# kylittle/Crucible

Hardware: AMD Instinct MI355X
Metric: Msamples/sec (whole node) + achieved HBM GB/s, book1 1920×1080 @ 1/2/4/8 GPU (higher is better)
Workload: dtype f64

## Files before the change

### crucible_amd/csrc/pathtrace.hpp

```cpp
#pragma once
#include <hip/hip_runtime.h>
#include <stddef.h>
#include <stdint.h>
#include <type_traits>

#define CR_HD __host__ __device__ __forceinline__
#define CR_D __device__ __forceinline__
#include "fastdiv.hpp"
#include "residency.hpp"

namespace cr {

template <typename real> struct RealTraits;
template <> struct RealTraits<float> {
    static constexpr float eps = 1.1920928955078125e-07f;
    static constexpr float tiny = 0.0f;
    static constexpr float pi = 3.14159265358979323846f;
};
template <> struct RealTraits<double> {
    static constexpr double eps = 2.220446049250313e-16;
    static constexpr double tiny = 1e-160;
    static constexpr double pi = 3.14159265358979323846;
};

// ... 599 lines not shown
    }
}
template <typename real> CR_D void random_in_unit_disk_dev(uint64_t& s, real& px, real& py) {
    if constexpr (!std::is_same<real, double>::value) {
        for (;;) {
            px = rng_range<real>(s, real(-1), real(1));
            py = rng_range<real>(s, real(-1), real(1));
            if (px * px + py * py + real(0) * real(0) < real(1)) break;
        }
    } else {
        uint64_t ux, uy;
        for (;;) {
            ux = rng_next(s); uy = rng_next(s);
            const float fx = screen_coord(ux), fy = screen_coord(uy);
            const float lf = __builtin_fmaf(fy, fy, fx * fx);
            if (lf > 1.0f + 1e-5f) continue;
            if (lf < 1.0f - 1e-5f) break;
            const double x = -1.0 + 2.0 * u01(ux, 0.0), y = -1.0 + 2.0 * u01(uy, 0.0);
            if (x * x + y * y + 0.0 * 0.0 < 1.0) break;
        }
        px = -1.0 + 2.0 * u01(ux, 0.0); py = -1.0 + 2.0 * u01(uy, 0.0);
    }
}

template <typename real, bool ANIM, bool CAMK = false>
CR_D void camera_ray(const KernelArgs<real>& A, uint32_t pix_i, uint32_t pix_j, int32_t sample, uint64_t& rng, V3<real>& ro, V3<real>& rd,
                     real& rtime, real current_time) {
    const CamConst<real>& cam = A.cam;
    uint32_t pixel = pix_j * (uint32_t)cam.W + pix_i;
    rng = rng_key(A.seed_mixed, pixel, (uint32_t)sample);
    real ts = current_time + rng_range<real>(rng, real(0), A.shutter_length);
    real ox = rng_uniform<real>(rng) - real(0.5);
    real oy = rng_uniform<real>(rng) - real(0.5);
    CamFrame<real> f;
    if ((ANIM || CAMK) && cam.animated) {
        real fx = cam.from.x, fy = cam.from.y, fz = cam.from.z, fw = real(1);
        real ax = cam.at.x, ay = cam.at.y, az = cam.at.z, aw = real(1);
        timeline_eval(A.cam_keys + cam.from_key_first, cam.from_key_count, ts, fx, fy, fz, fw);
        timeline_eval(A.cam_keys + cam.at_key_first, cam.at_key_count, ts, ax, ay, az, aw);
        f = camera_frame(cam, mk<real>(fw * fx, fw * fy, fw * fz), mk<real>(aw * ax, aw * ay, aw * az));
    } else {
        f.from = cam.from; f.p00 = cam.p00; f.pdu = cam.pdu; f.pdv = cam.pdv; f.ddu = cam.ddu; f.ddv = cam.ddv;
    }
    V3<real> ps = add(add(f.p00, scale((real)pix_i + ox, f.pdu)), scale((real)pix_j + oy, f.pdv));
    V3<real> orig = f.from;
    if (cam.defocus_on) {
        real px, py;
        random_in_unit_disk_dev<real>(rng, px, py);
        orig = add(add(f.from, scale(px, f.ddu)), scale(py, f.ddv));
    }
    ro = orig; rd = sub(ps, orig); rtime = ts;
}
template <typename real, bool ANIM, bool CAMK = false>
CR_D void camera_ray(const KernelArgs<real>& A, uint32_t pix_i, uint32_t pix_j, int32_t sample, uint64_t& rng, V3<real>& ro, V3<real>& rd,
                     real& rtime) {
    camera_ray<real, ANIM, CAMK>(A, pix_i, pix_j, sample, rng, ro, rd, rtime, A.current_time);
}

template <typename T> CR_D T load_rec(const T* p, bool in_lds) {
    static_assert(sizeof(T) % 4 == 0, "records are whole words");
    T out;
    uint32_t* o = reinterpret_cast<uint32_t*>(&out);
    if (in_lds) {
        const __attribute__((address_space(3))) uint32_t* s = (const __attribute__((address_space(3))) uint32_t*)(const void*)p;
        for (size_t k = 0; k < sizeof(T) / 4; k++) o[k] = s[k];
    } else {
        const __attribute__((address_space(1))) uint32_t* s = (const __attribute__((address_space(1))) uint32_t*)(const void*)p;
        for (size_t k = 0; k < sizeof(T) / 4; k++) o[k] = s[k];
    }
    return out;
}

#define CR_CHECKER_LEAF(tex_at, ti, tx, p)                                                                                          \
    for (int guard = 0; guard < 32 && tx.kind == 1; guard++) {                                                                   \
        int32_t s = (int32_t)((uint32_t)as_i32(r_floor(tx.inv_scale * p.x)) + (uint32_t)as_i32(r_floor(tx.inv_scale * p.y)) +   \
                              (uint32_t)as_i32(r_floor(tx.inv_scale * p.z)));                                                      \
        ti = (s % 2 == 0) ? tx.even : tx.odd;                                                                                    \
        tx = tex_at(ti);                                                                                                         \
    }

template <typename real, bool ANIM, bool SIDE_SPLIT = false, bool RELAX = false>
CR_D bool shade(const KernelArgs<real>& A, const Prim<real>* prims, const Mat<real>* mats, const Tex<real>* texs, V3<real>& ro, V3<real>& rd,
                real rtime, uint64_t& rng, int32_t& depth_left, int32_t& stack_n, real best_t, int32_t best, uint32_t stack_stride,
                uint32_t stack_slot, uint32_t& c_tex, V3<real>& col, Diag* dg = nullptr, V3<real>* thr = nullptr) {
    CR_DIAG_HIT(dg, DG_SHADE_WAVE, DG_SHADE_LANE);
    if (best >= 0) {
        CR_DIAG_HIT(dg, DG_HITSH_WAVE, DG_HITSH_LANE);
        const Prim<real>& p = prims[best];
        V3<real> loc = add(ro, scale(best_t, rd));
        V3<real> n;
        real tu = 0, tv = 0;
        auto mat_at = [&](int32_t i) { return SIDE_SPLIT ? load_rec(mats + i, A.lds_side != 0) : mats[i]; };
        auto tex_at = [&](int32_t i) { return SIDE_SPLIT ? load_rec(texs + i, A.lds_side != 0) : texs[i]; };
        const Mat<real> m = mat_at(p.mat());
        bool need_uv = false;
        int32_t leaf_tex = -1;
        if (m.kind == 0 && m.tex >= 0) {
            int ti = m.tex;
            Tex<real> tx = tex_at(ti);
            CR_CHECKER_LEAF(tex_at, ti, tx, loc)
            need_uv = tx.kind == 2;
            leaf_tex = ti;
        }
        if (p.kind() == 0) {
            real g0 = p.g[0], g1 = p.g[1], g2 = p.g[2], g3 = p.g[3];
            if (ANIM && p.key_count) {
                timeline_eval(A.keys + p.key_first, p.key_count, rtime, g0, g1, g2, g3);
                n = divs(sub(loc, mk<real>(g0, g1, g2)), g3);
            } else n = scale(p.g[4], sub(loc, mk<real>(g0, g1, g2)));
            if (need_uv) {
                real theta = r_acos(-n.y);
                real phi = r_atan2(-n.z, n.x) + RealTraits<real>::pi;
                tu = phi / (real(2) * RealTraits<real>::pi);
                tv = theta / RealTraits<real>::pi;
            }
        } else {
            V3<real> a = mk<real>(p.g[0], p.g[1], p.g[2]), b = mk<real>(p.g[3], p.g[4], p.g[5]), c = mk<real>(p.g[6], p.g[7], p.g[8]);
            if (ANIM && p.key_count) {
                a = timeline_vertex(A.keys + p.key_first, p.key_count, rtime, a);
                b = timeline_vertex(A.keys + p.key_first, p.key_count, rtime, b);
                c = timeline_vertex(A.keys + p.key_first, p.key_count, rtime, c);
            }
            n = unit(cross(sub(b, a), sub(c, a)));
            tu = 0; tv = 0;
        }
        bool front = dot(rd, n) < real(0);
        if (!front) n = neg(n);

        V3<real> att = mk<real>(0, 0, 0), ndir = rd;
        bool some;
        V3<real> ruv = mk<real>(0, 0, 0);
#ifdef CR_DIAG
        if (m.kind != 2) {
            for (;;) {
                CR_DIAG_HIT(dg, DG_RUV_WAVE, DG_RUV_LANE);
                real x = rng_range<real>(rng, real(-1), real(1)), y = rng_range<real>(rng, real(-1), real(1)), z = rng_range<real>(rng, real(-1), real(1));
                V3<real> pp = mk<real>(x, y, z);
                real lensq = len2(pp);
                if (RealTraits<real>::tiny < lensq && lensq <= real(1)) { ruv = divs(pp, r_sqrt(lensq)); break; }
            }
        }
        CR_DIAG_LANE(dg, m.kind == 0 ? DG_LAMB_LANE : (m.kind == 1 ? DG_METAL_LANE : DG_DIEL_LANE));
#else
        if (m.kind != 2) ruv = random_unit_vector_dev<real>(rng);
#endif
        if (m.kind == 0) {
            V3<real> dir = add(n, ruv);
            real tol = real(1e-8);
            if (r_abs(dir.x) < tol && r_abs(dir.y) < tol && r_abs(dir.z) < tol) dir = n;
            V3<real> tc;
            if (m.tex < 0) tc = mk<real>(m.albedo[0], m.albedo[1], m.albedo[2]);
            else {
                const Tex<real> lt = tex_at(leaf_tex);
                if (need_uv) tc = image_lookup(A.images, A.texels, lt.image, tu, tv, c_tex);
                else tc = mk<real>(lt.color[0], lt.color[1], lt.color[2]);
            }
            att = c_scale(m.aux, (m.param < real(0)) ? c_neg(tc) : tc);
            ndir = dir;
            if (__ballot(!(m.param >= real(1))) == 0ull) { rng_step(rng); some = true; }
            else some = rng_uniform<real>(rng) <= m.param;
        } else if (m.kind == 1) {
            V3<real> refl = reflect(rd, n);
            refl = add(unit(refl), scale(m.param, ruv));
            att = mk<real>(m.albedo[0], m.albedo[1], m.albedo[2]);
            ndir = refl;
            some = dot(refl, n) > real(0);
        } else {
            att = mk<real>(1, 1, 1);
            real ri = front ? m.albedo[0] : m.param;
            V3<real> ud = unit(rd);
            real cos_theta = -(r_fmin(dot(ud, n), real(1)));
            real sin_theta = r_sqrt(real(1) - cos_theta * cos_theta);
            bool refl = ri * sin_theta > real(1);
            if (!refl) {
                real r0 = front ? m.albedo[1] : m.albedo[2];
                real x = real(1) - cos_theta;
                real x2 = x * x;
                real x5 = x * (x2 * x2);
                refl = (r0 + (real(1) - r0) * x5) > rng_uniform<real>(rng);
            }
            ndir = refl ? reflect(ud, n) : refract(ud, n, ri);
            some = true;
        }
        if (!some) { col = mk<real>(0, 0, 0); return true; }
        if (m.kind != 2) {
            if constexpr (RELAX) { thr->x = thr->x * att.x; thr->y = thr->y * att.y; thr->z = thr->z * att.z; }
            else {
                real* rec = A.att_stack + ((size_t)stack_n * stack_stride + stack_slot) * 3;
                rec[0] = att.x; rec[1] = att.y; rec[2] = att.z;
                stack_n++;
            }
        }
        ro = loc; rd = ndir; depth_left--;
        return false;
    }
    CR_DIAG_LANE(dg, DG_SKY_LANE);
    V3<real> ud = unit(rd);
    if (A.sky_kind == 1) {
        real theta = r_atan2(ud.x, ud.z);
        real phi = r_asin(ud.y);
        real u = (theta / (real(2) * RealTraits<real>::pi)) + real(0.5);
        real v = (phi / RealTraits<real>::pi) + real(0.5);
        col = image_lookup(A.images, A.texels, A.sky_image, u, v, c_tex);
    } else {
        real a = real(0.5) * (ud.y + real(1));
        col = c_add(c_scale(real(1) - a, mk<real>(1, 1, 1)), c_scale(a, mk<real>(real(0.5), real(0.7), real(1))));
    }
    if constexpr (RELAX) { col = mk<real>(thr->x * col.x, thr->y * col.y, thr->z * col.z); return true; }
    int32_t k = stack_n - 1;
    for (; k >= 3; k -= 4) {
        CR_DIAG_HIT(dg, DG_UNWIND_WAVE, DG_UNWIND_LANE);
        V3<real> a[4];
#pragma unroll
        for (int j = 0; j < 4; j++) {
            const real* rec = A.att_stack + ((size_t)(k - j) * stack_stride + stack_slot) * 3;
            a[j] = mk<real>(rec[0], rec[1], rec[2]);
        }
#pragma unroll
        for (int j = 0; j < 4; j++) col = c_mul(a[j], col);
    }
    for (; k >= 0; k--) {
        CR_DIAG_HIT(dg, DG_UNWIND_WAVE, DG_UNWIND_LANE);
        const real* rec = A.att_stack + ((size_t)k * stack_stride + stack_slot) * 3;
        V3<real> a_k = mk<real>(rec[0], rec[1], rec[2]);
        col = c_mul(a_k, col);
    }
    return true;
}

template <typename T> using LdsPtr = const __attribute__((address_space(3))) T*;
template <typename T> using GlobPtr = const __attribute__((address_space(1))) T*;
template <typename real, int RES>
CR_D Entry<real> fetch_entry(const Entry<real>* lds, const Entry<real>* glob, int32_t lds_entries, int32_t idx) {
    if (RES == RES_LDS) return lds[idx];
    if (RES == RES_TOP) {
        Entry<real> e;
        if (idx < lds_entries) {
            const Entry<real>* s = lds + idx;
            LdsPtr<real> b = (LdsPtr<real>)s->b;
            for (int k = 0; k < 6; k++) e.b[k] = b[k];
            e.skip = *(LdsPtr<int32_t>)&s->skip; e.leaf = *(LdsPtr<int32_t>)&s->leaf;
        } else {
            const Entry<real>* s = glob + idx;
            GlobPtr<real> b = (GlobPtr<real>)s->b;
            for (int k = 0; k < 6; k++) e.b[k] = b[k];
            e.skip = *(GlobPtr<int32_t>)&s->skip; e.leaf = *(GlobPtr<int32_t>)&s->leaf;
        }
        return e;
    }
    return glob[idx];
}
template <typename real, int RES>
CR_D Entry<real> fetch_entry_ordered(const Entry<real>* lds, const Entry<real>* glob, int32_t lds_entries, int32_t idx, int32_t oct) {
    auto rd = [&](const EntryO<real>* p) {
        const EntryO<real>& s = p[idx];
        Entry<real> e;
        for (int k = 0; k < 6; k++) e.b[k] = s.b[k];
        e.leaf = s.leaf;
        e.skip = s.skip[oct];
        return e;
    };
    if (RES == RES_LDS) return rd((const EntryO<real>*)lds);
    if (RES == RES_TOP) {
        Entry<real> e;
        if (idx < lds_entries) {
            const EntryO<real>* s = (const EntryO<real>*)lds + idx;
            LdsPtr<real> b = (LdsPtr<real>)s->b;
            for (int k = 0; k < 6; k++) e.b[k] = b[k];
            e.leaf = *(LdsPtr<int32_t>)&s->leaf; e.skip = ((LdsPtr<int32_t>)s->skip)[oct];
        } else {
            const EntryO<real>* s = (const EntryO<real>*)glob + idx;
            GlobPtr<real> b = (GlobPtr<real>)s->b;
            for (int k = 0; k < 6; k++) e.b[k] = b[k];
            e.leaf = *(GlobPtr<int32_t>)&s->leaf; e.skip = ((GlobPtr<int32_t>)s->skip)[oct];
        }
        return e;
    }
    return rd((const EntryO<real>*)glob);
}

template <int RES> CR_D uint32_t screen_lds_base(const void* lds) { return RES == RES_LDS ? (uint32_t)(uintptr_t)(LdsPtr<char>)lds : 0u; }
template <int RES>
CR_D ScreenEntry fetch_screen(const ScreenEntry* lds, const ScreenEntry* glob, uint32_t lds_bytes, uint32_t off) {
    static_assert(sizeof(ScreenEntry) == 32, "offsets are index << 5");
    typedef uint32_t Quad __attribute__((ext_vector_type(4)));
    if (RES == RES_LDS) {
        ScreenEntry e;
        Quad* o = reinterpret_cast<Quad*>(&e);
        LdsPtr<Quad> s = (LdsPtr<Quad>)(uintptr_t)off;
        o[0] = s[0]; o[1] = s[1];
        return e;
    }
    if (RES == RES_TOP) {
        ScreenEntry e;
        Quad* o = reinterpret_cast<Quad*>(&e);
        if (off < lds_bytes) {
            LdsPtr<Quad> s = (LdsPtr<Quad>)(const void*)((const char*)lds + off);
            o[0] = s[0]; o[1] = s[1];
        } else {
            GlobPtr<Quad> s = (GlobPtr<Quad>)(const void*)((const char*)glob + off);
            o[0] = s[0]; o[1] = s[1];
        }
        return e;
    }
    return *(const ScreenEntry*)((const char*)glob + off);
}

struct ScreenStepO { float b[6]; uint32_t axis, hit, skip; };
template <int RES>
CR_D ScreenStepO fetch_screen_ordered(const ScreenEntryO* lds, const ScreenEntryO* glob, uint32_t lds_bytes, uint32_t off, uint32_t octoff) {
    static_assert(sizeof(ScreenEntryO) == 64, "offsets are index << 6");
    typedef uint32_t Quad __attribute__((ext_vector_type(4)));
    ScreenStepO e;
    Quad q0, q1;
    if (RES == RES_LDS) {
        LdsPtr<Quad> s = (LdsPtr<Quad>)(uintptr_t)off;
        q0 = s[0]; q1 = s[1];
        e.skip = *(LdsPtr<uint32_t>)(uintptr_t)(off + octoff);
    } else if (RES == RES_TOP && off < lds_bytes) {
        LdsPtr<Quad> s = (LdsPtr<Quad>)(const void*)((const char*)lds + off);
        q0 = s[0]; q1 = s[1];
        e.skip = *(LdsPtr<uint32_t>)(const void*)((const char*)lds + off + octoff);
    } else {
        GlobPtr<Quad> s = (GlobPtr<Quad>)(const void*)((const char*)glob + off);
        q0 = s[0]; q1 = s[1];
        e.skip = *(GlobPtr<uint32_t>)(const void*)((const char*)glob + off + octoff);
    }
    uint32_t w[8];
    __builtin_memcpy(w, &q0, 16); __builtin_memcpy(w + 4, &q1, 16);
    for (int k = 0; k < 6; k++) e.b[k] = __builtin_bit_cast(float, w[k]);
    e.axis = w[6]; e.hit = w[7];
    return e;
}

template <typename real> struct WalkState {
    V3<real> inv;
    real dd;
    real rda;
    real best_t;
    int32_t best;
    int32_t idx;
    bool exact_box;
    int32_t oct;
    int32_t pending;
};

CR_D bool tree_walks_exact(const KernelArgs<float>& A) { return A.exact_boxes != 0; }
CR_D constexpr bool tree_walks_exact(const KernelArgs<double>&) { return false; }

template <bool SHARED = false, typename real> CR_D void walk_begin(WalkState<real>& w, V3<real> rd, bool exact_tree = false) {
    w.inv = mk<real>(real(1) / rd.x, real(1) / rd.y, real(1) / rd.z);
    w.exact_box = exact_tree || (r_abs(w.inv.x) == r_inf(real(0))) || (r_abs(w.inv.y) == r_inf(real(0))) || (r_abs(w.inv.z) == r_inf(real(0)));
    w.dd = len2(rd);
    w.rda = SHARED ? shared_rcp(w.dd) : quot_divide<real>();
    w.idx = 0; w.best_t = r_inf(real(0)); w.best = -1; w.pending = -1;
    w.oct = (rd.x < real(0) ? 1 : 0) | (rd.y < real(0) ? 2 : 0) | (rd.z < real(0) ? 4 : 0);
}

CR_D void screen_extents(float ofx, float ofy, float ofz, float ifx, float ify, float ifz, float& mo, float& pmax, float& pmin) {
    mo = r_max(r_max(__builtin_fabsf(ofx), __builtin_fabsf(ofy)), __builtin_fabsf(ofz));
    pmax = r_max(r_max(__builtin_fabsf(ifx), __builtin_fabsf(ify)), __builtin_fabsf(ifz));
    pmin = r_min(r_min(__builtin_fabsf(ifx), __builtin_fabsf(ify)), __builtin_fabsf(ifz));
}
CR_D bool screen_in_range(bool exact_box, float mo, float pmax, float pmin) {
    return !exact_box && pmin >= 0x1.0p-100f && pmax <= 0x1.0p100f && mo <= 0x1.0p100f;
}
CR_D float screen_q(float of, float inv_f) { return __builtin_fabsf(of * inv_f); }
CR_D float screen_th0(float qx, float qy, float qz, float pmax) {
    return __builtin_fmaf(0x1.0p-20f, r_max(r_max(qx, qy), qz), __builtin_fmaf(pmax * 0x1.0p-100f, 0x1.0p-47f, 1e-35f));
}
CR_D float screen_box_d(const float* b, Pair<float> fox, Pair<float> foy, Pair<float> foz, Pair<float> fix, Pair<float> fiy, Pair<float> fiz,
                        float tminf, float tmaxf, float th0, float& th) {
    const Pair<float> tx = __builtin_elementwise_fma(Pair<float>{b[0], b[1]}, fix, -(fox * fix));
    const Pair<float> ty = __builtin_elementwise_fma(Pair<float>{b[2], b[3]}, fiy, -(foy * fiy));
    const Pair<float> tz = __builtin_elementwise_fma(Pair<float>{b[4], b[5]}, fiz, -(foz * fiz));
    const float nx = r_min(tx.x, tx.y), ny = r_min(ty.x, ty.y), nz = r_min(tz.x, tz.y);
    const float fx = r_max(tx.x, tx.y), fy = r_max(ty.x, ty.y), fz = r_max(tz.x, tz.y);
    const float lo = r_max(r_max(nx, ny), r_max(nz, tminf));
    float hi, m;
    asm("v_min_f32_e32 %0, %2, %3\n\tv_min3_f32 %0, %4, %5, %0\n\tv_max_f32_e64 %1, |%6|, |%0|"
        : "=&v"(hi), "=v"(m) : "v"(fz), "v"(tmaxf), "v"(fx), "v"(fy), "v"(lo));
    th = __builtin_fmaf(0x1.0p-20f, m, th0);
    return hi - lo;
}
CR_D bool screen_box_miss_exact(const float* b, Pair<float> fox, Pair<float> foy, Pair<float> foz, Pair<float> fix, Pair<float> fiy,
                                Pair<float> fiz, float tminf, float tmaxf) {
    const Pair<float> tx = (Pair<float>{b[0], b[1]} - fox) * fix;
    const Pair<float> ty = (Pair<float>{b[2], b[3]} - foy) * fiy;
    const Pair<float> tz = (Pair<float>{b[4], b[5]} - foz) * fiz;
    const float nx = r_min(tx.x, tx.y), ny = r_min(ty.x, ty.y), nz = r_min(tz.x, tz.y);
    const float fx = r_max(tx.x, tx.y), fy = r_max(ty.x, ty.y), fz = r_max(tz.x, tz.y);
    const float lo = r_max(r_max(nx, ny), r_max(nz, tminf));
    float hi;
    asm("v_min_f32_e32 %0, %1, %2\n\tv_min3_f32 %0, %3, %4, %0" : "=&v"(hi) : "v"(fz), "v"(tmaxf), "v"(fx), "v"(fy));
    return hi <= lo;
}

template <typename real, int RES, bool ANIM, bool SCREEN> constexpr int quot_form() {
    constexpr bool fits = std::is_same<real, double>::value && !ANIM && SCREEN && RES != RES_GLOBAL;
#ifdef CR_QUOT_FORM
    return fits ? CR_QUOT_FORM : 0;
#else
    return fits ? 1 : 0;
#endif
}

template <typename real, int RES, bool ANIM, bool ORD = false, bool SCREEN = false, bool SHARE = false>
CR_D void walk_round(const KernelArgs<real>& A, const Entry<real>* lds_entries, const Prim<real>* prims, V3<real> ro, V3<real> rd, real rtime,
                     WalkState<real>& w, bool walking, uint32_t budget, unsigned long long& c_node, uint32_t& c_prim, Diag* dg = nullptr,
                     const void* lds_screen = nullptr) {
    constexpr bool EXACT = std::is_same<real, float>::value;
    static_assert(!(SCREEN && EXACT && ORD), "the f32 kernels use ScreenEntry records for unordered trees only");
    const real tmin = real(0.001);
    const int32_t n_entries = A.n_entries;
    constexpr int RES64 = SCREEN ? RES_GLOBAL : RES;
    const int32_t lds_n64 = SCREEN ? 0 : A.lds_entries;
    int32_t leaf = w.pending;
    if (walking && leaf < 0) {
        CR_DIAG_HIT(dg, DG_ROUND_WAVE, DG_ROUND_LANE);
        uint32_t exact_steps = w.exact_box ? 0xffffffffu : 0u;
        if constexpr (SCREEN) {
            const float ofx = (float)ro.x, ofy = (float)ro.y, ofz = (float)ro.z;
            const float ifx = (float)w.inv.x, ify = (float)w.inv.y, ifz = (float)w.inv.z;
            float mo, pmax, pmin;
            screen_extents(ofx, ofy, ofz, ifx, ify, ifz, mo, pmax, pmin);
            bool screened;
            if constexpr (EXACT) screened = !w.exact_box;
            else screened = screen_in_range(w.exact_box, mo, pmax, pmin);
            if (!screened) exact_steps = 0xffffffffu;
            else {
                const float qx = screen_q(ofx, ifx), qy = screen_q(ofy, ify), qz = screen_q(ofz, ifz);
                const Pair<float> fox = {ofx, ofx}, foy = {ofy, ofy}, foz = {ofz, ofz};
                const Pair<float> fix = {ifx, ifx}, fiy = {ify, ify}, fiz = {ifz, ifz};
                const float tminf = 0.001f;
                float tmaxf = (float)w.best_t;
                const float th0 = screen_th0(qx, qy, qz, pmax);
                asm volatile("" : "+v"(tmaxf));
                uint32_t nodes = 0;
                auto box_miss = [&](const float* b, int32_t idx) -> bool {
                    if constexpr (EXACT) {
                        const bool miss = screen_box_miss_exact(b, fox, foy, foz, fix, fiy, fiz, tminf, tmaxf);
                        nodes++;
                        CR_DIAG_HIT(dg, DG_BOX_WAVE, DG_BOX_LANE);
                        return miss;
                    }
                    float th;
                    float d = screen_box_d(b, fox, foy, foz, fix, fiy, fiz, tminf, tmaxf, th0, th);
                    nodes++;
                    CR_DIAG_HIT(dg, DG_BOX_WAVE, DG_BOX_LANE);
                    const bool band = !(__builtin_fabsf(d) > th);
                    if (__builtin_expect(__ballot(band) != 0ull, 0)) {
                        if (band) {
                            CR_DIAG_HIT(dg, DG_BAND_WAVE, DG_BAND_LANE);
                            const Entry<real> e = ORD ? fetch_entry_ordered<real, RES64>(lds_entries, A.entries, lds_n64, idx, w.oct)
                                                      : fetch_entry<real, RES64>(lds_entries, A.entries, lds_n64, idx);
                            d = box_hit(e.b, ro, w.inv, tmin, w.best_t) ? 1.0f : -1.0f;
                        }
                    }
                    return d < 0.0f;
                };
                if constexpr (ORD) {
                    const uint32_t base = screen_lds_base<RES>(lds_screen);
                    const uint32_t end = base + ((uint32_t)n_entries << 6);
                    const uint32_t oct = (uint32_t)w.oct, octoff = 32u + (oct << 2);
                    uint32_t off = base + ((uint32_t)w.idx << 6), after_leaf = 0;
                    if (off < end) {
                        for (uint32_t it = 0;; it++) {
                            const ScreenStepO se = fetch_screen_ordered<RES>((const ScreenEntryO*)lds_screen, (const ScreenEntryO*)A.screen, (uint32_t)A.lds_entries << 6, off, octoff);
                            const bool miss = box_miss(se.b, (int32_t)((off - base) >> 6));
                            after_leaf = se.skip;
                            off = miss ? se.skip : se.hit + (__builtin_amdgcn_ubfe(oct, se.axis, 1u) << 6);
                            uint32_t limit = (it + 1 == budget) ? 0u : end;
                            asm("" : "+s"(limit));
                            if (off >= limit) break;
                        }
                        if (off & kScreenLeaf) { leaf = (int32_t)(off & ~kScreenLeaf); off = after_leaf; }
                        w.idx = (int32_t)((off - base) >> 6);
                    }
                } else {
                    const uint32_t base = screen_lds_base<RES>(lds_screen);
                    const uint32_t end = base + ((uint32_t)n_entries << 5);
                    uint32_t off = base + ((uint32_t)w.idx << 5), after_leaf = 0;
                    if (off < end) {
                        for (uint32_t it = 0;; it++) {
                            const ScreenEntry se = fetch_screen<RES>((const ScreenEntry*)lds_screen, (const ScreenEntry*)A.screen, (uint32_t)A.lds_entries << 5, off);
                            const bool miss = box_miss(se.b, (int32_t)((off - base) >> 5));
                            after_leaf = se.skip;
                            off = miss ? se.skip : se.hit;
                            uint32_t limit = (it + 1 == budget) ? 0u : end;
                            asm("" : "+s"(limit));
                            if (off >= limit) break;
                        }
                        if (off & kScreenLeaf) { leaf = (int32_t)(off & ~kScreenLeaf); off = after_leaf; }
                        w.idx = (int32_t)((off - base) >> 5);
                    }
                }
                c_node += nodes;
            }
        } else if (!w.exact_box) {
            const Pair<real> ox = {ro.x, ro.x}, oy = {ro.y, ro.y}, oz = {ro.z, ro.z};
            const Pair<real> ix = {w.inv.x, w.inv.x}, iy = {w.inv.y, w.inv.y}, iz = {w.inv.z, w.inv.z};
            const real tmax = w.best_t;
            uint32_t nodes = 0;
            for (uint32_t it = 0; w.idx < n_entries; it++) {
                const Entry<real> e = ORD ? fetch_entry_ordered<real, RES64>(lds_entries, A.entries, lds_n64, w.idx, w.oct)
                                          : fetch_entry<real, RES64>(lds_entries, A.entries, lds_n64, w.idx);
                nodes++;
                CR_DIAG_HIT(dg, DG_BOX_WAVE, DG_BOX_LANE);
                const bool miss = box_miss_fast(e.b, ox, oy, oz, ix, iy, iz, tmin, tmax);
                const bool inner = e.leaf < 0;
                w.idx = (inner && !miss) ? (ORD ? ordered_near(e.leaf, w.oct) : -e.leaf) : e.skip;
                if (!(miss || inner)) { leaf = e.leaf; break; }
                if (it + 1 == budget) break;
            }
            c_node += nodes;
        }
        for (; exact_steps != 0u && w.idx < n_entries; exact_steps--) {
            const Entry<real> e = ORD ? fetch_entry_ordered<real, RES64>(lds_entries, A.entries, lds_n64, w.idx, w.oct)
                                      : fetch_entry<real, RES64>(lds_entries, A.entries, lds_n64, w.idx);
            c_node++;
            bool hit = box_hit(e.b, ro, w.inv, tmin, w.best_t);
            w.idx = (hit && e.leaf < 0) ? (ORD ? ordered_near(e.leaf, w.oct) : -e.leaf) : e.skip;
            if (hit && e.leaf >= 0) { leaf = e.leaf; break; }
        }
    }
    w.pending = leaf;
    if (A.walk_leaf_min > 0u) {
        const uint32_t parked = (uint32_t)__popcll(__ballot(leaf >= 0));
        const bool can_step = __ballot(walking && leaf < 0 && w.idx < n_entries) != 0ull;
        if (parked < A.walk_leaf_min && can_step) return;
    }
    w.pending = -1;
    if (leaf >= 0) {
        CR_DIAG_HIT(dg, DG_LEAFPH_WAVE, DG_LEAFPH_LANE);
        constexpr int QF = SHARE ? quot_form<real, RES, ANIM, SCREEN>() : 0;
        const real ra = QF == 1 ? w.rda : (QF == 2 ? shared_rcp(w.dd) : quot_divide<real>());
        auto test = [&](int32_t pi) {
            const Prim<real>& p = prims[pi];
            c_prim++;
            CR_DIAG_HIT(dg, DG_PRIM_WAVE, DG_PRIM_LANE);
            real t;
            bool h;
            real g0 = p.g[0], g1 = p.g[1], g2 = p.g[2], g3 = p.g[3];
            const int32_t kind = A.uniform_kind >= 0 ? A.uniform_kind : p.kind();
            if (kind == 0) {
                if (ANIM && p.key_count) timeline_eval(A.keys + p.key_first, p.key_count, rtime, g0, g1, g2, g3);
                h = sphere_t<RES == RES_LDS || (std::is_same<real, double>::value && !ANIM), QF != 0>(g0, g1, g2, g3, ro, rd, w.dd, tmin, w.best_t, t, dg, ra);
            } else {
                V3<real> a = mk<real>(g0, g1, g2), b = mk<real>(g3, p.g[4], p.g[5]), c = mk<real>(p.g[6], p.g[7], p.g[8]);
                if (ANIM && p.key_count) {
                    a = timeline_vertex(A.keys + p.key_first, p.key_count, rtime, a);
                    b = timeline_vertex(A.keys + p.key_first, p.key_count, rtime, b);
                    c = timeline_vertex(A.keys + p.key_first, p.key_count, rtime, c);
                }
                h = triangle_t(a, b, c, ro, rd, tmin, w.best_t, t);
            }
            if (h) { w.best_t = t; w.best = pi; }
        };
        if (!ANIM || A.leaf_runs == nullptr || !(leaf & kLeafRun)) {
            const int32_t first = leaf >> 1, count = (leaf & 1) + 1;
            if constexpr (RES != RES_LDS && !ANIM) {
                constexpr uint32_t touch = sizeof(Prim<real>) == 96 ? 20u : (uint32_t)(sizeof(Prim<real>) / 4 - 1);
                static_assert((touch + 1) * 4 <= sizeof(Prim<real>), "the touched word must lie inside the record");
                GlobPtr<uint32_t> nx = (GlobPtr<uint32_t>)(const void*)(prims + first + (count - 1));
                const uint32_t t0 = nx[0], t1 = nx[touch];
                test(first);
                asm volatile("" :: "v"(t0), "v"(t1));
                if (count == 2) test(first + 1);
            } else
            for (int32_t k = 0; k < count; k++) test(first + k);
        } else {
            const int32_t first = A.leaf_runs[2 * (leaf & kLeafRunIndex)], count = A.leaf_runs[2 * (leaf & kLeafRunIndex) + 1];
            for (int32_t k = 0; k < count; k++) test(first + k);
        }
    }
}

#ifdef CR_DIAG
#define CR_DIAG_ONLY(...) __VA_ARGS__
#else
#define CR_DIAG_ONLY(...)
#endif

enum : int { ST_NEED_PIXEL = 0, ST_NEED_SAMPLE = 1, ST_TRACE = 2, ST_DONE = 3, ST_WALK = 4, ST_SHADE = 5 };

template <typename real> struct MaxBlock { static constexpr int value = 1024; };

CR_D uint32_t wave_rank(uint64_t ballot) {
    return __builtin_amdgcn_mbcnt_hi((uint32_t)(ballot >> 32), __builtin_amdgcn_mbcnt_lo((uint32_t)ballot, 0u));
}

template <typename real> CR_D const KernelArgs<real>& kernel_args() {
    return *(const KernelArgs<real>*)(const __attribute__((address_space(4))) KernelArgs<real>*)__builtin_amdgcn_kernarg_segment_ptr();
}
template <typename real, int RES, bool ANIM, bool ORD, bool CAMK = false, bool RELAX = false, bool SCREEN = false, bool REG = true, bool LIST = false>
CR_D void pathtrace_body(const KernelArgs<real>& A) {
    using EntryT = typename EntryOf<real, ORD>::type;
    constexpr bool BATCH = RELAX && (ANIM || CAMK);
    constexpr bool REGION = BATCH && REG;
    const KernelArgs<real>& RG = kernel_args<real>();
    extern __shared__ __attribute__((aligned(16))) unsigned char smem[];
#ifdef CR_HOLD_VCC
    unsigned long long vcc_hold;
    asm volatile("s_mov_b64 %0, 0" : "={vcc}"(vcc_hold));
#endif
    const Entry<real>* lds_entries = nullptr;
    const void* lds_screen = nullptr;
    const Prim<real>* prims = A.prims;
    const Mat<real>* mats = A.mats;
    const Tex<real>* texs = A.texs;
    if (RES != RES_GLOBAL) {
        auto copy = [&](const void* src, size_t off, size_t bytes) {
            const uint32_t* s = (const uint32_t*)src;
            uint32_t* d = (uint32_t*)(smem + off);
            for (size_t i = threadIdx.x; i < bytes / 4; i += blockDim.x) d[i] = s[i];
        };
        using ScreenT = typename ScreenOf<ORD>::type;
        constexpr size_t window_rec = SCREEN ? sizeof(ScreenT) : sizeof(EntryT);
        copy(SCREEN ? A.screen : (const void*)A.entries, 0, (size_t)A.lds_entries * window_rec);
        lds_entries = (const Entry<real>*)smem;
        if (SCREEN) lds_screen = (const void*)smem;
        if (RES == RES_LDS) {
            size_t o1 = (((size_t)A.n_entries * window_rec + 15) & ~(size_t)15);
            size_t o2 = o1 + (((size_t)A.n_prims * sizeof(Prim<real>) + 15) & ~(size_t)15);
            size_t o3 = o2 + (((size_t)A.n_mats * sizeof(Mat<real>) + 15) & ~(size_t)15);
            copy(A.prims, o1, (size_t)A.n_prims * sizeof(Prim<real>));
            copy(A.mats, o2, (size_t)A.n_mats * sizeof(Mat<real>));
            copy(A.texs, o3, (size_t)A.n_texs * sizeof(Tex<real>));
            prims = (const Prim<real>*)(smem + o1);
            mats = (const Mat<real>*)(smem + o2);
            texs = (const Tex<real>*)(smem + o3);
            if constexpr (SCREEN) {
                __syncthreads();
                const uint32_t base = screen_lds_base<RES>(smem);
                ScreenT* rec = (ScreenT*)smem;
                for (int32_t i = (int32_t)threadIdx.x; i < A.n_entries; i += (int32_t)blockDim.x) {
                    if constexpr (ORD) { for (int k = 0; k < 8; k++) rec[i].skip[k] += base; }
                    else rec[i].skip += base;
                    if (!(rec[i].hit & kScreenLeaf)) rec[i].hit += base;
                }
            }
        } else if (A.lds_side) {
            size_t o2 = (((size_t)A.lds_entries * window_rec + 15) & ~(size_t)15);
            size_t o3 = o2 + (((size_t)A.n_mats * sizeof(Mat<real>) + 15) & ~(size_t)15);
            copy(A.mats, o2, (size_t)A.n_mats * sizeof(Mat<real>));
            copy(A.texs, o3, (size_t)A.n_texs * sizeof(Tex<real>));
            mats = (const Mat<real>*)(smem + o2);
            texs = (const Tex<real>*)(smem + o3);
        }
        __syncthreads();
    }

    const uint32_t lane = threadIdx.x & 63u;
    const uint32_t gtid = blockIdx.x * blockDim.x + threadIdx.x;
    constexpr uint32_t kFxNoTile = 0xffffffffu;
    unsigned long long* fx_slots = nullptr;
    uint32_t fx_tile0 = kFxNoTile, fx_tile1 = kFxNoTile, fx_mru = 0;
    V3<real> thr = mk<real>(1, 1, 1);
    const uint32_t fx_words = 3u << (A.sg_lw + A.sg_lh);
    if constexpr (RELAX) {
        fx_slots = (unsigned long long*)(smem + A.fx_lds_off) + (size_t)(threadIdx.x >> 6) * 2 * fx_words;
        for (uint32_t k = lane; k < 2 * fx_words; k += 64) fx_slots[k] = 0ull;
        __builtin_amdgcn_fence(__ATOMIC_SEQ_CST, "wavefront");
    }
    auto fx_flush = [&](uint32_t slot, uint32_t tile) {
        if constexpr (RELAX) {
            __builtin_amdgcn_fence(__ATOMIC_SEQ_CST, "wavefront");
            if (tile != kFxNoTile) {
                uint32_t ti, tj;
                tile_xy(A, tile, ti, tj);
                ti <<= A.sg_lw; tj <<= A.sg_lh;
                if constexpr (BATCH) tj -= batch_frame(A, tj) * ((A.tiles_y << A.sg_lh) - (REGION ? RG.reg_h : (uint32_t)A.cam.H));
                for (uint32_t k = lane; k < fx_words; k += 64) {
                    unsigned long long* w = fx_slots + slot * fx_words + k;
                    const unsigned long long v = *w;
                    if (v) {
                        *w = 0ull;
                        const uint32_t px = k / 3u, ch = k - px * 3u;
                        const uint32_t pi = ti + (px & ((1u << A.sg_lw) - 1u)), pj = tj + (px >> A.sg_lw);
                        unsigned long long* g;
                        if constexpr (REGION) g = A.fx_acc + ((size_t)pj * (size_t)RG.reg_w + pi) * 3 + ch;
                        else g = A.fx_acc + ((size_t)pj * (size_t)A.cam.W + pi) * 3 + ch;
                        if (v & ~kFxNaN) atomicAdd(g, v & ~kFxNaN);
                        if (v & kFxNaN) atomicOr(g, kFxNaN);
                    }
                }
            }
            __builtin_amdgcn_fence(__ATOMIC_SEQ_CST, "wavefront");
        }
    };
    const uint32_t total_work = (A.sg_on || RELAX) ? A.sg_total : A.tiles_x * A.tiles_y * 64u;
    const CamConst<real>& cam = A.cam;
    uint32_t wv_next = 0, wv_end = 0;
    const uint32_t SG_CHUNK = A.sg_chunk;

    int state = ST_NEED_PIXEL;
    uint32_t pix_i = 0, pix_j = 0;
    uint32_t item = 0;
    int32_t sample = 0;
    real acc_r = 0, acc_g = 0, acc_b = 0;
    V3<real> ro = mk<real>(0, 0, 0), rd = mk<real>(0, 0, 1);
    real rtime = 0;
    uint64_t rng = 0;
    int32_t depth_left = 0, stack_n = 0;
    uint32_t c_seg = 0, c_prim = 0, c_tex = 0;
    unsigned long long c_node = 0;
    WalkState<real> ws;
    ws.inv = mk<real>(0, 0, 0); ws.dd = 0; ws.rda = quot_divide<real>(); ws.best_t = 0; ws.best = -1; ws.idx = 0; ws.exact_box = false; ws.pending = -1;
    const int32_t n_entries = A.n_entries;
    uint32_t exact_tree = tree_walks_exact(A) ? 1u : 0u;
    if constexpr (std::is_same<real, float>::value) {
        exact_tree = (uint32_t)__builtin_amdgcn_readfirstlane((int)exact_tree);
        asm volatile("" : "+s"(exact_tree));
    }

    Diag* dgp = nullptr;
    CR_DIAG_ONLY(Diag dg_store; for (int i = 0; i < DG_N; i++) dg_store.v[i] = 0; dgp = &dg_store;
                 unsigned long long d_t_regen = 0, d_t_trace = 0, d_t_shade = 0;
                 unsigned long long d_t0 = __builtin_readcyclecounter(); const unsigned long long d_begin = d_t0;)
    for (;;) {
        CR_DIAG_ONLY(if (CR_DIAG_LEADER()) dg_store.v[DG_OUTER_WAVE]++; d_t0 = __builtin_readcyclecounter();)
        uint64_t need = __ballot(state == ST_NEED_PIXEL);
        if (need && (A.sg_on || RELAX)) {
            const uint32_t cnt = (uint32_t)__popcll(need), avail = wv_end - wv_next;
            uint32_t fresh = 0;
            uint32_t my_tile = kFxNoTile;
            if (cnt > avail) {
                const int leader = __ffsll((unsigned long long)need) - 1;
                if ((int)lane == leader) fresh = atomicAdd(A.work_counter, SG_CHUNK);
                fresh = (uint32_t)__builtin_amdgcn_readlane((int)fresh, leader);
            }
            if (state == ST_NEED_PIXEL) {
                const uint32_t rank = wave_rank(need);
                const uint32_t w = rank < avail ? wv_next + rank : fresh + (rank - avail);
                if (w >= total_work) state = ST_DONE;
                else {
                    item = w;
                    const uint32_t group = w >> 6, in = w & 63u;
                    uint32_t tile = fastdiv(group, A.fd_groups);
                    const uint32_t sg = group - tile * A.sg_groups;
                    if constexpr (REGION && LIST) { const int32_t* const listed = RG.tile_list; if (listed) tile = (uint32_t)listed[tile]; }
                    uint32_t tx, ty;
                    tile_xy(A, tile, tx, ty);
                    my_tile = tile;
                    const uint32_t px = in & ((1u << A.sg_lw) - 1u), py = (in >> A.sg_lw) & ((1u << A.sg_lh) - 1u);
                    const uint32_t ds = in >> (A.sg_lw + A.sg_lh);
                    pix_i = (tx << A.sg_lw) + px;
                    pix_j = (ty << A.sg_lh) + py;
                    const uint32_t s_off = sg * (64u >> (A.sg_lw + A.sg_lh)) + ds;
                    sample = (int32_t)((uint32_t)A.sample_begin + s_off);
                    uint32_t row = pix_j;
                    if constexpr (BATCH) row -= batch_frame(A, pix_j) * (A.tiles_y << A.sg_lh);
                    bool inside;
                    if constexpr (REGION) inside = pix_i < RG.reg_w && row < RG.reg_h;
                    else inside = pix_i < (uint32_t)cam.W && row < (uint32_t)cam.H;
                    if (inside && s_off < (uint32_t)(A.sample_end - A.sample_begin)) state = ST_NEED_SAMPLE;
                    if constexpr (REGION) { pix_i += RG.reg_x0; pix_j += RG.reg_y0; }
                }
            }
            if (cnt > avail) { wv_next = fresh + (cnt - avail); wv_end = fresh + SG_CHUNK; }
            else wv_next += cnt;
            if constexpr (RELAX) {
                uint64_t fresh_items = __ballot(state == ST_NEED_SAMPLE) & need;
                while (fresh_items) {
                    const uint32_t t = (uint32_t)__builtin_amdgcn_readlane((int)my_tile, __ffsll((unsigned long long)fresh_items) - 1);
                    fresh_items &= ~__ballot(my_tile == t);
                    if (t == fx_tile0) fx_mru = 0;
                    else if (t == fx_tile1) fx_mru = 1;
                    else if (fx_mru == 0) { fx_flush(1, fx_tile1); fx_tile1 = t; fx_mru = 1; }
                    else { fx_flush(0, fx_tile0); fx_tile0 = t; fx_mru = 0; }                }
            }
        } else if (need) {
            uint32_t cnt = (uint32_t)__popcll(need);
            uint32_t base = 0;
            int leader = __ffsll((unsigned long long)need) - 1;
            if ((int)lane == leader) base = atomicAdd(A.work_counter, cnt);
            base = (uint32_t)__builtin_amdgcn_readlane((int)base, leader);
            if (state == ST_NEED_PIXEL) {
                uint32_t rank = wave_rank(need);
                uint32_t w = base + rank;
                if (w >= total_work) state = ST_DONE;
                else {
                    uint32_t tile = w >> 6, in = w & 63u;
                    uint32_t tx, ty;
                    tile_xy(A, tile, tx, ty);
                    pix_i = tx * 8u + (in & 7u);
                    pix_j = ty * 8u + (in >> 3);
                    if (pix_i < (uint32_t)cam.W && pix_j < (uint32_t)cam.H) {
                        state = ST_NEED_SAMPLE; sample = A.sample_begin; acc_r = acc_g = acc_b = 0;
                    }
                }
            }
        }
        if (__ballot(state != ST_DONE) == 0) break;

        if (state == ST_NEED_SAMPLE) {
            CR_DIAG_HIT(dgp, DG_REGEN_WAVE, DG_REGEN_LANE);
            if constexpr (BATCH) {
                const uint32_t f = batch_frame(A, REGION ? pix_j - RG.reg_y0 : pix_j);
                camera_ray<real, ANIM, CAMK>(A, pix_i, pix_j - f * (A.tiles_y << A.sg_lh), sample, rng, ro, rd, rtime,
                                             A.n_frames > 1u ? A.frame_times[f] : A.current_time);
            } else camera_ray<real, ANIM, CAMK>(A, pix_i, pix_j, sample, rng, ro, rd, rtime);
            depth_left = A.max_depth; stack_n = 0;
            if constexpr (RELAX) thr = mk<real>(1, 1, 1);
            state = ST_TRACE;
        }

        CR_DIAG_ONLY({ unsigned long long t = __builtin_readcyclecounter(); d_t_regen += t - d_t0; d_t0 = t; })
        V3<real> col = mk<real>(0, 0, 0);
        bool finished = false;
        if (state == ST_TRACE) {
            if (depth_left == 0) finished = true;
            else {
                c_seg++;
                walk_begin<quot_form<real, RES, ANIM, SCREEN>() == 1>(ws, rd, exact_tree != 0u);
                state = n_entries > 0 ? ST_WALK : ST_SHADE;
            }
        }
        if (__ballot(state == ST_WALK)) {
            for (;;) {
                walk_round<real, RES, ANIM, ORD, SCREEN, true>(A, lds_entries, prims, ro, rd, rtime, ws, state == ST_WALK, A.walk_round_steps, c_node, c_prim, dgp, lds_screen);
                if (state == ST_WALK && ws.idx >= n_entries && ws.pending < 0) state = ST_SHADE;
                const uint64_t walking = __ballot(state == ST_WALK);
                if (!walking || 64u - (uint32_t)__popcll(walking) >= A.walk_exit_lanes) break;
            }
        }
        const bool tracing = (state == ST_SHADE);

        CR_DIAG_ONLY({ unsigned long long t = __builtin_readcyclecounter(); d_t_trace += t - d_t0; d_t0 = t; })
        if (tracing) {
            finished = shade<real, ANIM, RES == RES_TOP, RELAX>(A, prims, mats, texs, ro, rd, rtime, rng, depth_left, stack_n, ws.best_t, ws.best,
                                         A.n_threads, gtid, c_tex, col, dgp, &thr);
            state = ST_TRACE;
        }

        if (RELAX && finished) {
            if constexpr (RELAX) {
                const bool black = col.x == real(0) && col.y == real(0) && col.z == real(0);
                if (!black) {
                    uint32_t ri = pix_i, rj = pix_j;
                    if constexpr (REGION) { ri -= RG.reg_x0; rj -= RG.reg_y0; }
                    const uint32_t tile = (rj >> A.sg_lh) * A.tiles_x + (ri >> A.sg_lw);
                    const uint32_t px = ((rj & ((1u << A.sg_lh) - 1u)) << A.sg_lw) | (ri & ((1u << A.sg_lw) - 1u));
                    const real cc[3] = {col.x, col.y, col.z};
                    unsigned long long v[3];
#pragma unroll
                    for (int c = 0; c < 3; c++) {
                        const double x = (double)cc[c];
                        v[c] = (x == x) ? (unsigned long long)(__builtin_bit_cast(long long, __builtin_fma(x, A.fx_scale, 0x1.0p52)) - 0x4330000000000000ll) : kFxNaN;
                    }
                    const bool nan = (v[0] | v[1] | v[2]) >> 63;
                    unsigned long long* dst;
                    bool in_lds = true;
                    if (tile == fx_tile0) dst = fx_slots + px * 3u;
                    else if (tile == fx_tile1) dst = fx_slots + fx_words + px * 3u;
                    else {
                        uint32_t row = rj;
                        if constexpr (BATCH) row -= batch_frame(A, rj) * ((A.tiles_y << A.sg_lh) - (REGION ? RG.reg_h : (uint32_t)cam.H));
                        if constexpr (REGION) dst = A.fx_acc + ((size_t)row * (size_t)RG.reg_w + ri) * 3;
                        else dst = A.fx_acc + ((size_t)row * (size_t)cam.W + ri) * 3;
                        in_lds = false;
                    }
                    if (!nan) {
                        if (in_lds) {
                            auto d = (__attribute__((address_space(3))) unsigned long long*)dst;
                            for (int c = 0; c < 3; c++) if (v[c]) (void)__hip_atomic_fetch_add(d + c, v[c], __ATOMIC_RELAXED, __HIP_MEMORY_SCOPE_WORKGROUP);
                        } else {
                            auto d = (__attribute__((address_space(1))) unsigned long long*)dst;
                            for (int c = 0; c < 3; c++) if (v[c]) (void)__hip_atomic_fetch_add(d + c, v[c], __ATOMIC_RELAXED, __HIP_MEMORY_SCOPE_AGENT);
                        }
                    } else {
                        for (int c = 0; c < 3; c++) {
                            if (v[c] >> 63) atomicOr(dst + c, kFxNaN);
                            else if (v[c]) atomicAdd(dst + c, v[c]);
                        }
                    }
                }
            }
            state = ST_NEED_PIXEL;
        } else if (finished && A.sg_on) {
            real* o = A.sample_buf + (size_t)item * 3;
            o[0] = col.x; o[1] = col.y; o[2] = col.z;
            state = ST_NEED_PIXEL;
        } else if (finished) {
            acc_r += col.x; acc_g += col.y; acc_b += col.z;
            sample++;
            if (sample >= A.sample_end) {
                size_t o = ((size_t)pix_j * (size_t)cam.W + pix_i) * 3;
                if (A.output_sum) { A.out[o] = acc_r; A.out[o + 1] = acc_g; A.out[o + 2] = acc_b; }
                else {
                    real cnt = (real)A.samples_total;
                    A.out[o] = acc_r / cnt; A.out[o + 1] = acc_g / cnt; A.out[o + 2] = acc_b / cnt;
                }
                state = ST_NEED_PIXEL;
            } else state = ST_NEED_SAMPLE;
        }
        CR_DIAG_ONLY({ unsigned long long t = __builtin_readcyclecounter(); d_t_shade += t - d_t0; d_t0 = t; })
    }

    if constexpr (RELAX) { fx_flush(0, fx_tile0); fx_flush(1, fx_tile1); }
    auto wave_sum = [&](unsigned long long v) -> unsigned long long {
        unsigned long long s = v;
        for (int off = 32; off > 0; off >>= 1) s += __shfl_down(s, off);
        return s;
    };
    unsigned long long s0 = wave_sum(c_seg), s1 = wave_sum(c_node), s2 = wave_sum(c_prim), s3 = wave_sum(c_tex);
    CR_DIAG_ONLY(
        {
            unsigned long long* c = (unsigned long long*)A.counters;
            for (int i = 0; i < DG_N; i++) { unsigned long long w = wave_sum(dg_store.v[i]); if (lane == 0) atomicAdd(&c[16 + i], w); }
            if (lane == 0) {
                atomicAdd(&c[9], d_t_regen); atomicAdd(&c[10], d_t_trace); atomicAdd(&c[11], d_t_shade);
                atomicAdd(&c[12], __builtin_readcyclecounter() - d_begin);
            }
        })
// ... 85 lines not shown
```

Measured before the change: 4832.

## Compute f64 ray inverse lazily, add sphere leaf loop, reuse squared length in shade

For the f64 screened kernels, the walk now keeps only a float reciprocal of the ray direction, computed with a hardware rcp plus one Newton step. The full double-precision inverse is recomputed on demand, only when exact box tests are needed, instead of being stored in the walk state. It also adds a specialised one-or-two-sphere leaf loop for LDS-resident uniform-sphere scenes. Shade now reuses the squared direction length from the walk state instead of renormalising the ray. The aims are fewer f64 divisions and lower register pressure, at the cost of more template variants and some recomputation on exact fallback paths.

```diff
diff --git a/crucible_amd/csrc/pathtrace.hpp b/crucible_amd/csrc/pathtrace.hpp
--- a/crucible_amd/csrc/pathtrace.hpp
+++ b/crucible_amd/csrc/pathtrace.hpp
@@ -705,8 +705,9 @@
 template <typename real, bool ANIM, bool SIDE_SPLIT = false, bool RELAX = false>
 CR_D bool shade(const KernelArgs<real>& A, const Prim<real>* prims, const Mat<real>* mats, const Tex<real>* texs, V3<real>& ro, V3<real>& rd,
                 real rtime, uint64_t& rng, int32_t& depth_left, int32_t& stack_n, real best_t, int32_t best, uint32_t stack_stride,
-                uint32_t stack_slot, uint32_t& c_tex, V3<real>& col, Diag* dg = nullptr, V3<real>* thr = nullptr) {
+                uint32_t stack_slot, uint32_t& c_tex, V3<real>& col, Diag* dg = nullptr, V3<real>* thr = nullptr, const real* dd = nullptr) {
     CR_DIAG_HIT(dg, DG_SHADE_WAVE, DG_SHADE_LANE);
+    auto unit_rd = [&]() -> V3<real> { return divs(rd, r_sqrt(dd ? *dd : len2(rd))); };
     if (best >= 0) {
         CR_DIAG_HIT(dg, DG_HITSH_WAVE, DG_HITSH_LANE);
         const Prim<real>& p = prims[best];
@@ -791,7 +792,7 @@
         } else {
             att = mk<real>(1, 1, 1);
             real ri = front ? m.albedo[0] : m.param;
-            V3<real> ud = unit(rd);
+            V3<real> ud = unit_rd();
             real cos_theta = -(r_fmin(dot(ud, n), real(1)));
             real sin_theta = r_sqrt(real(1) - cos_theta * cos_theta);
             bool refl = ri * sin_theta > real(1);
@@ -818,7 +819,7 @@
         return false;
     }
     CR_DIAG_LANE(dg, DG_SKY_LANE);
-    V3<real> ud = unit(rd);
+    V3<real> ud = unit_rd();
     if (A.sky_kind == 1) {
         real theta = r_atan2(ud.x, ud.z);
         real phi = r_asin(ud.y);
@@ -956,7 +957,12 @@
     return e;
 }
 
-template <typename real> struct WalkState {
+template <typename real> struct WalkScreened {};
+template <> struct WalkScreened<double> {
+    V3<float> invf;
+    bool unscreened;
+};
+template <typename real> struct WalkState : WalkScreened<real> {
     V3<real> inv;
     real dd;
     real rda;
@@ -979,6 +985,7 @@
     w.idx = 0; w.best_t = r_inf(real(0)); w.best = -1; w.pending = -1;
     w.oct = (rd.x < real(0) ? 1 : 0) | (rd.y < real(0) ? 2 : 0) | (rd.z < real(0) ? 4 : 0);
 }
+template <bool SHARED = false, typename real> CR_D void walk_begin_screened(WalkState<real>& w, V3<real> ro, V3<real> rd);
 
 CR_D void screen_extents(float ofx, float ofy, float ofz, float ifx, float ify, float ifz, float& mo, float& pmax, float& pmin) {
     mo = r_max(r_max(__builtin_fabsf(ofx), __builtin_fabsf(ofy)), __builtin_fabsf(ofz));
@@ -988,9 +995,30 @@
 CR_D bool screen_in_range(bool exact_box, float mo, float pmax, float pmin) {
     return !exact_box && pmin >= 0x1.0p-100f && pmax <= 0x1.0p100f && mo <= 0x1.0p100f;
 }
+CR_D double screen_rcp1(double d) {
+    const double r0 = __builtin_amdgcn_rcp(d);
+    return __builtin_fma(r0, __builtin_fma(-d, r0, 1.0), r0);
+}
+CR_D float screen_inv(double d) { return (float)screen_rcp1(d); }
+CR_D float screen_inv(float d) { return 1.0f / d; }
+CR_D bool screen_in_range_lazy(float mo, float ifx, float ify, float ifz) {
+    const float ax = __builtin_fabsf(ifx), ay = __builtin_fabsf(ify), az = __builtin_fabsf(ifz);
+    return ax >= 0x1.0p-100f && ax <= 0x1.0p100f && ay >= 0x1.0p-100f && ay <= 0x1.0p100f && az >= 0x1.0p-100f && az <= 0x1.0p100f &&
+           mo <= 0x1.0p100f;
+}
 CR_D float screen_q(float of, float inv_f) { return __builtin_fabsf(of * inv_f); }
 CR_D float screen_th0(float qx, float qy, float qz, float pmax) {
     return __builtin_fmaf(0x1.0p-20f, r_max(r_max(qx, qy), qz), __builtin_fmaf(pmax * 0x1.0p-100f, 0x1.0p-47f, 1e-35f));
+}
+template <bool SHARED, typename real> CR_D void walk_begin_screened(WalkState<real>& w, V3<real> ro, V3<real> rd) {
+    static_assert(std::is_same<real, double>::value, "the f32 kernels' record is the wrapper's own box: they begin with walk_begin");
+    w.invf = mk<float>(screen_inv(rd.x), screen_inv(rd.y), screen_inv(rd.z));
+    const float mo = r_max(r_max(__builtin_fabsf((float)ro.x), __builtin_fabsf((float)ro.y)), __builtin_fabsf((float)ro.z));
+    w.unscreened = !screen_in_range_lazy(mo, w.invf.x, w.invf.y, w.invf.z);
+    w.dd = len2(rd);
+    w.rda = SHARED ? shared_rcp(w.dd) : quot_divide<real>();
+    w.idx = 0; w.best_t = r_inf(real(0)); w.best = -1; w.pending = -1;
+    w.oct = (rd.x < real(0) ? 1 : 0) | (rd.y < real(0) ? 2 : 0) | (rd.z < real(0) ? 4 : 0);
 }
 CR_D float screen_box_d(const float* b, Pair<float> fox, Pair<float> foy, Pair<float> foz, Pair<float> fix, Pair<float> fiy, Pair<float> fiz,
                         float tminf, float tmaxf, float th0, float& th) {
@@ -1028,12 +1056,35 @@
 #endif
 }
 
-template <typename real, int RES, bool ANIM, bool ORD = false, bool SCREEN = false, bool SHARE = false>
+#ifndef CR_SPHERE_LOOP
+#define CR_SPHERE_LOOP 1
+#endif
+#ifndef CR_SHADE_DD
+#define CR_SHADE_DD 1
+#endif
+template <typename real, int RES, bool ANIM, bool ORD, bool CAMK, bool SCREEN> constexpr bool lazy_inv() {
+#if defined(CR_LAZY_INV) && CR_LAZY_INV == 0
+    return false;
+#else
+    return std::is_same<real, double>::value && SCREEN && !ANIM && !ORD && !CAMK;
+#endif
+}
+template <typename real, int RES, bool ANIM, bool ORD, bool CAMK, bool SCREEN> constexpr bool sphere_loop() {
+    return CR_SPHERE_LOOP && std::is_same<real, double>::value && SCREEN && RES == RES_LDS && !ANIM && !ORD && !CAMK;
+}
+
+template <typename real> CR_D V3<real> inv_of(V3<real> rd) {
+    asm volatile("" : "+v"(rd.x), "+v"(rd.y), "+v"(rd.z));
+    return mk<real>(real(1) / rd.x, real(1) / rd.y, real(1) / rd.z);
+}
+
+template <typename real, int RES, bool ANIM, bool ORD = false, bool SCREEN = false, bool SHARE = false, bool LAZY_INV = false, bool SPHERE_LOOP = false>
 CR_D void walk_round(const KernelArgs<real>& A, const Entry<real>* lds_entries, const Prim<real>* prims, V3<real> ro, V3<real> rd, real rtime,
                      WalkState<real>& w, bool walking, uint32_t budget, unsigned long long& c_node, uint32_t& c_prim, Diag* dg = nullptr,
                      const void* lds_screen = nullptr) {
     constexpr bool EXACT = std::is_same<real, float>::value;
     static_assert(!(SCREEN && EXACT && ORD), "the f32 kernels use ScreenEntry records for unordered trees only");
+    static_assert(!LAZY_INV || (SCREEN && !EXACT), "LAZY_INV is a form of the f64 SCREEN kernels");
     const real tmin = real(0.001);
     const int32_t n_entries = A.n_entries;
     constexpr int RES64 = SCREEN ? RES_GLOBAL : RES;
@@ -1041,14 +1092,19 @@
     int32_t leaf = w.pending;
     if (walking && leaf < 0) {
         CR_DIAG_HIT(dg, DG_ROUND_WAVE, DG_ROUND_LANE);
-        uint32_t exact_steps = w.exact_box ? 0xffffffffu : 0u;
+        uint32_t exact_steps = 0u;
+        if constexpr (!LAZY_INV) exact_steps = w.exact_box ? 0xffffffffu : 0u;
         if constexpr (SCREEN) {
             const float ofx = (float)ro.x, ofy = (float)ro.y, ofz = (float)ro.z;
-            const float ifx = (float)w.inv.x, ify = (float)w.inv.y, ifz = (float)w.inv.z;
+            float ifx, ify, ifz;
+            if constexpr (LAZY_INV) { ifx = w.invf.x; ify = w.invf.y; ifz = w.invf.z; }
+            else { ifx = (float)w.inv.x; ify = (float)w.inv.y; ifz = (float)w.inv.z; }
             float mo, pmax, pmin;
-            screen_extents(ofx, ofy, ofz, ifx, ify, ifz, mo, pmax, pmin);
+            if constexpr (LAZY_INV) pmax = r_max(r_max(__builtin_fabsf(ifx), __builtin_fabsf(ify)), __builtin_fabsf(ifz));
+            else screen_extents(ofx, ofy, ofz, ifx, ify, ifz, mo, pmax, pmin);
             bool screened;
-            if constexpr (EXACT) screened = !w.exact_box;
+            if constexpr (LAZY_INV) screened = !w.unscreened;
+            else if constexpr (EXACT) screened = !w.exact_box;
             else screened = screen_in_range(w.exact_box, mo, pmax, pmin);
             if (!screened) exact_steps = 0xffffffffu;
             else {
@@ -1077,7 +1133,8 @@
                             CR_DIAG_HIT(dg, DG_BAND_WAVE, DG_BAND_LANE);
                             const Entry<real> e = ORD ? fetch_entry_ordered<real, RES64>(lds_entries, A.entries, lds_n64, idx, w.oct)
                                                       : fetch_entry<real, RES64>(lds_entries, A.entries, lds_n64, idx);
-                            d = box_hit(e.b, ro, w.inv, tmin, w.best_t) ? 1.0f : -1.0f;
+                            if constexpr (LAZY_INV) d = box_hit(e.b, ro, inv_of(rd), tmin, w.best_t) ? 1.0f : -1.0f;
+                            else d = box_hit(e.b, ro, w.inv, tmin, w.best_t) ? 1.0f : -1.0f;
                         }
                     }
                     return d < 0.0f;
@@ -1138,11 +1195,15 @@
             }
             c_node += nodes;
         }
+        V3<real> inv_lazy = mk<real>(0, 0, 0);
+        if constexpr (LAZY_INV) { if (exact_steps != 0u && w.idx < n_entries) inv_lazy = inv_of(rd); }
         for (; exact_steps != 0u && w.idx < n_entries; exact_steps--) {
             const Entry<real> e = ORD ? fetch_entry_ordered<real, RES64>(lds_entries, A.entries, lds_n64, w.idx, w.oct)
                                       : fetch_entry<real, RES64>(lds_entries, A.entries, lds_n64, w.idx);
             c_node++;
-            bool hit = box_hit(e.b, ro, w.inv, tmin, w.best_t);
+            bool hit;
+            if constexpr (LAZY_INV) hit = box_hit(e.b, ro, inv_lazy, tmin, w.best_t);
+            else hit = box_hit(e.b, ro, w.inv, tmin, w.best_t);
             w.idx = (hit && e.leaf < 0) ? (ORD ? ordered_near(e.leaf, w.oct) : -e.leaf) : e.skip;
             if (hit && e.leaf >= 0) { leaf = e.leaf; break; }
         }
@@ -1190,6 +1251,22 @@
                 test(first);
                 asm volatile("" :: "v"(t0), "v"(t1));
                 if (count == 2) test(first + 1);
+            } else if constexpr (SPHERE_LOOP) {
+                static_assert(RES == RES_LDS && !ANIM, "the one-or-two-record loop on primitives in LDS");
+                if (A.uniform_kind == 0) {
+                    auto sphere = [&](int32_t pi) {
+                        const Prim<real>& p = prims[pi];
+                        c_prim++;
+                        CR_DIAG_HIT(dg, DG_PRIM_WAVE, DG_PRIM_LANE);
+                        real t;
+                        if (sphere_t<true, QF != 0>(p.g[0], p.g[1], p.g[2], p.g[3], ro, rd, w.dd, tmin, w.best_t, t, dg, ra)) { w.best_t = t; w.best = pi; }
+                    };
+                    sphere(first);
+                    if (leaf & 1) sphere(first + 1);
+                } else {
+                    test(first);
+                    if (leaf & 1) test(first + 1);
+                }
             } else
             for (int32_t k = 0; k < count; k++) test(first + k);
         } else {
@@ -1330,6 +1407,8 @@
     unsigned long long c_node = 0;
     WalkState<real> ws;
     ws.inv = mk<real>(0, 0, 0); ws.dd = 0; ws.rda = quot_divide<real>(); ws.best_t = 0; ws.best = -1; ws.idx = 0; ws.exact_box = false; ws.pending = -1;
+    constexpr bool LAZY = lazy_inv<real, RES, ANIM, ORD, CAMK, SCREEN>();
+    if constexpr (LAZY) { ws.invf = mk<float>(0, 0, 0); ws.unscreened = false; }
     const int32_t n_entries = A.n_entries;
     uint32_t exact_tree = tree_walks_exact(A) ? 1u : 0u;
     if constexpr (std::is_same<real, float>::value) {
@@ -1436,13 +1515,14 @@
             if (depth_left == 0) finished = true;
             else {
                 c_seg++;
-                walk_begin<quot_form<real, RES, ANIM, SCREEN>() == 1>(ws, rd, exact_tree != 0u);
+                if constexpr (LAZY) walk_begin_screened<quot_form<real, RES, ANIM, SCREEN>() == 1>(ws, ro, rd);
+                else walk_begin<quot_form<real, RES, ANIM, SCREEN>() == 1>(ws, rd, exact_tree != 0u);
                 state = n_entries > 0 ? ST_WALK : ST_SHADE;
             }
         }
         if (__ballot(state == ST_WALK)) {
             for (;;) {
-                walk_round<real, RES, ANIM, ORD, SCREEN, true>(A, lds_entries, prims, ro, rd, rtime, ws, state == ST_WALK, A.walk_round_steps, c_node, c_prim, dgp, lds_screen);
+                walk_round<real, RES, ANIM, ORD, SCREEN, true, LAZY, sphere_loop<real, RES, ANIM, ORD, CAMK, SCREEN>()>(A, lds_entries, prims, ro, rd, rtime, ws, state == ST_WALK, A.walk_round_steps, c_node, c_prim, dgp, lds_screen);
                 if (state == ST_WALK && ws.idx >= n_entries && ws.pending < 0) state = ST_SHADE;
                 const uint64_t walking = __ballot(state == ST_WALK);
                 if (!walking || 64u - (uint32_t)__popcll(walking) >= A.walk_exit_lanes) break;
@@ -1453,7 +1533,7 @@
         CR_DIAG_ONLY({ unsigned long long t = __builtin_readcyclecounter(); d_t_trace += t - d_t0; d_t0 = t; })
         if (tracing) {
             finished = shade<real, ANIM, RES == RES_TOP, RELAX>(A, prims, mats, texs, ro, rd, rtime, rng, depth_left, stack_n, ws.best_t, ws.best,
-                                         A.n_threads, gtid, c_tex, col, dgp, &thr);
+                                         A.n_threads, gtid, c_tex, col, dgp, &thr, CR_SHADE_DD ? &ws.dd : nullptr);
             state = ST_TRACE;
         }
 
```

After: 4938, median of 6. 2.2% higher.
